# stm233/image-compression-for-machine

Hardware: AMD Instinct MI355X
Metric: images/sec (256x256) cnn-hyperprior (WACNN) training step (higher is better)
Workload: dtype f32; 1 GPU; cnn (WACNN N=192 M=320) train step, lambda=0.0067 MSE, batch 16/GPU synthetic 256x256, Adam lr 1e-4 + aux Adam, clip 1.0; global_batch=16, parallelism=dp1

## Files before the change

### image-compression-for-machine_amd/csrc/conv_wino.hip

```cpp
#include <cmath>
#include <cstdlib>
#include "conv_common.h"

namespace icm {

struct WinoDesc {
  ConvPtrs g[ICM_MAX_GROUPS];
  long long x_bs, y_bs, res_bs, aux_bs, y2_bs;
  int N, Cin, Cout, H, W;
  int lgTX, lgTY, lgTI, tiles_x, tiles_y, tiles_n;
  int ncot, nchunks8, ncb, nsteps;
  int epi, accum, act;
  int seg_len, seg_gap;
  FastDiv dseg;
  int dbg;
  int vpre;
  int px_fast, npx;
};

#define WINO_STEP_FLOATS (2 * 16 * 8 * 32)

template <int EPI>
__device__ __forceinline__ void wino_finish(const WinoDesc& d, const ConvPtrs& P, float v, int co, long long off, bool ok) {
  if (!ok) return;
  if (P.bias) v += P.bias[co];
  float side;
  v = epi_apply<EPI>(v, epi_reads_res(EPI) ? P.res[off] : 0.0f, epi_reads_aux(EPI) ? P.aux[off] : 0.0f, side);
  if constexpr (epi_writes_side(EPI))
    if (P.y2) P.y2[off] = side;
  if (d.accum) v += P.y[off];
  if constexpr (epi_may_gelu(EPI))
    if (P.y2) epi_materialise(v, P.y, P.y2, off, true);
  P.y[off] = v;
}

typedef float f32x2 __attribute__((ext_vector_type(2)));
template <int EPI>
__device__ __forceinline__ void wino_finish2(const WinoDesc& d, const ConvPtrs& P, float v0, float v1, int co, long long off,
                                             bool ok) {
  if (!ok) return;
  if (P.bias) {
    const float b = P.bias[co];
    v0 += b;
    v1 += b;
  }
  f32x2 rv = {0.0f, 0.0f}, av = {0.0f, 0.0f};
  if constexpr (epi_reads_res(EPI)) rv = *reinterpret_cast<const f32x2*>(P.res + off);
  if constexpr (epi_reads_aux(EPI)) av = *reinterpret_cast<const f32x2*>(P.aux + off);
  float s0, s1;
  v0 = epi_apply<EPI>(v0, rv[0], av[0], s0);
  v1 = epi_apply<EPI>(v1, rv[1], av[1], s1);
  if constexpr (epi_writes_side(EPI))
    if (P.y2) *reinterpret_cast<f32x2*>(P.y2 + off) = f32x2{s0, s1};
  if (d.accum) {
    const f32x2 old = *reinterpret_cast<const f32x2*>(P.y + off);
    v0 += old[0];
    v1 += old[1];
  }
  if constexpr (epi_may_gelu(EPI))
    if (P.y2) {
      float g0 = v0, g1 = v1;
      epi_materialise(g0, P.y, P.y, off, false);
      epi_materialise(g1, P.y, P.y, off, false);
      if (P.y2 == P.y) {
        v0 = g0;
        v1 = g1;
      } else {
        *reinterpret_cast<f32x2*>(P.y2 + off) = f32x2{g0, g1};
      }
    }
  *reinterpret_cast<f32x2*>(P.y + off) = f32x2{v0, v1};
}

template <int TCO>
__global__ __launch_bounds__(512, 2) void conv_wino_kernel(const WinoDesc d) {
  extern __shared__ __attribute__((aligned(16))) float smem[];
  const int tid = threadIdx.x, lane = tid & 63;
  const int wave = __builtin_amdgcn_readfirstlane(tid >> 6);
  ConvPtrs P = d.g[blockIdx.y];
  int bid = xcd_block_id();
  const int cb = d.px_fast ? bid / d.npx : bid % d.ncb;
  int pt = d.px_fast ? bid % d.npx : bid / d.ncb;
  const int pblk = pt;
  const int bx = pt % d.tiles_x;
  pt /= d.tiles_x;
  const int by = pt % d.tiles_y;
  const int bn = pt / d.tiles_y;
  const int TXm = (1 << d.lgTX) - 1, TYm = (1 << d.lgTY) - 1;
  const int HW = d.H * d.W;

  if (wave >= 4 && d.vpre) {
    const int lw = wave - 4;
    const float* vsrc = P.x + (long long)pblk * (d.nsteps * 2) * 4096;
    auto dma = [&](int step, int buf) {
#pragma unroll
      for (int k = 0; k < 2; ++k)
#pragma unroll
        for (int rnd = 0; rnd < 4; ++rnd) {
          const int e = (rnd * 256 + lw * 64) * 4;
          __builtin_amdgcn_global_load_lds(vsrc + ((long long)(step * 2 + k) * 4096 + e + lane * 4),
                                           smem + buf * WINO_STEP_FLOATS + k * 4096 + e, 16, 0, 0);
        }
    };
    dma(0, 0);
    asm volatile("s_waitcnt vmcnt(0)" ::: "memory");
    __syncthreads();
    for (int s = 0; s < d.nsteps; ++s) {
      if (s + 1 < d.nsteps) dma(s + 1, (s + 1) & 1);
      asm volatile("s_waitcnt vmcnt(0)" ::: "memory");
      __syncthreads();
    }
  } else if (wave >= 4) {
    const int q = (wave - 4) * 64 + lane;
    const int ci_l = q >> 5, t = q & 31;
    const int tx = t & TXm, ty = (t >> d.lgTX) & TYm, ti = t >> (d.lgTX + d.lgTY);
    const int n = (bn << d.lgTI) + ti;
    const int oy = (((by << d.lgTY) + ty) << 1), ox = (((bx << d.lgTX) + tx) << 1);
    unsigned mask = 0;
#pragma unroll
    for (int dy = 0; dy < 4; ++dy)
#pragma unroll
      for (int dx = 0; dx < 4; ++dx) {
        const int iy = oy - 1 + dy, ix = ox - 1 + dx;
        if (n < d.N && (unsigned)iy < (unsigned)d.H && (unsigned)ix < (unsigned)d.W) mask |= 1u << (dy * 4 + dx);
      }
    const float* xbase = P.x + ((long long)n * d.x_bs + (long long)(oy - 1) * d.W + (ox - 1));
    const int act = d.act;
    auto load = [&](float (&r)[2][16], int step) {
#pragma unroll
      for (int k = 0; k < 2; ++k) {
        const int c = (step * 2 + k) * 8 + ci_l;
        const bool cok = c < d.Cin;
        const int cp = d.seg_len ? c + (int)fdiv((uint32_t)c, d.dseg) * d.seg_gap : c;
        const float* pc = xbase + (long long)cp * HW;
#pragma unroll
        for (int dy = 0; dy < 4; ++dy)
#pragma unroll
          for (int dx = 0; dx < 4; ++dx)
            r[k][dy * 4 + dx] = (cok && ((mask >> (dy * 4 + dx)) & 1u) && !(d.dbg & 1)) ? pc[dy * d.W + dx] : 0.0f;
      }
    };
    auto transform_store = [&](const float (&r)[2][16], int buf) {
      if (d.dbg & 8) return;
#pragma unroll
      for (int k = 0; k < 2; ++k) {
        float dd[16], u[16];
#pragma unroll
        for (int e = 0; e < 16; ++e) dd[e] = act ? apply_act(r[k][e], act) : r[k][e];
#pragma unroll
        for (int j = 0; j < 4; ++j) {
          u[0 * 4 + j] = dd[0 * 4 + j] - dd[2 * 4 + j];
          u[1 * 4 + j] = dd[1 * 4 + j] + dd[2 * 4 + j];
          u[2 * 4 + j] = dd[2 * 4 + j] - dd[1 * 4 + j];
          u[3 * 4 + j] = dd[1 * 4 + j] - dd[3 * 4 + j];
        }
        float* dst = smem + buf * WINO_STEP_FLOATS + k * (16 * 256) + ci_l * 32 + t;
#pragma unroll
        for (int i = 0; i < 4; ++i) {
          dst[(i * 4 + 0) * 256] = u[i * 4 + 0] - u[i * 4 + 2];
          dst[(i * 4 + 1) * 256] = u[i * 4 + 1] + u[i * 4 + 2];
          dst[(i * 4 + 2) * 256] = u[i * 4 + 2] - u[i * 4 + 1];
          dst[(i * 4 + 3) * 256] = u[i * 4 + 1] - u[i * 4 + 3];
        }
      }
    };
    float ra[2][16], rb[2][16], rc[2][16];
    load(ra, 0);
    if (d.nsteps > 1) load(rb, 1);
    if (d.nsteps > 2) load(rc, 2);
    transform_store(ra, 0);
    __syncthreads();
    for (int s = 0; s < d.nsteps; s += 3) {
      if (s + 3 < d.nsteps) load(ra, s + 3);
      if (s + 1 < d.nsteps) transform_store(rb, (s + 1) & 1);
      __syncthreads();
      if (s + 1 >= d.nsteps) break;
      if (s + 4 < d.nsteps) load(rb, s + 4);
      if (s + 2 < d.nsteps) transform_store(rc, (s + 2) & 1);
      __syncthreads();
      if (s + 2 >= d.nsteps) break;
      if (s + 5 < d.nsteps) load(rc, s + 5);
      if (s + 3 < d.nsteps) transform_store(ra, (s + 3) & 1);
      __syncthreads();
    }
  } else {
  const int r = wave;
  f32x16 acc[4][TCO];
  const int cot0 = cb * TCO;
#pragma unroll
  for (int c = 0; c < 4; ++c)
#pragma unroll
    for (int a = 0; a < TCO; ++a)
#pragma unroll
      for (int e = 0; e < 16; ++e) acc[c][a][e] = 0.0f;
  const char* wbase = reinterpret_cast<const char*>(P.wp);
  unsigned wl[TCO];
#pragma unroll
  for (int a = 0; a < TCO; ++a) wl[a] = (unsigned)(min(cot0 + a, d.ncot - 1) * 64 + lane) * 16u;
  const long long qstride = (long long)d.ncot * 64 * 16;
  const int nunits = d.nsteps * 8;
  const int lastq = d.nchunks8 * 16 - 1;
  auto wptr = [&](int g) -> const char* {
    const int qq = min((g >> 2) * 16 + 4 * r + (g & 3), lastq);
    return wbase + qq * qstride;
  };
  f32x4 aq[4][TCO];
#pragma unroll
  for (int u = 0; u < 3; ++u)
#pragma unroll
    for (int a = 0; a < TCO; ++a) aq[u][a] = *reinterpret_cast<const f32x4*>(wptr(u) + wl[a]);
  const int boff = (4 * r) * 256 + lane;
  __syncthreads();
  for (int s = 0; s < d.nsteps; ++s) {
    const float* vb = smem + (s & 1) * WINO_STEP_FLOATS + boff;
    float bv[2][4];
#pragma unroll
    for (int j = 0; j < 4; ++j) bv[0][j] = vb[j * 64];
#pragma unroll
    for (int u = 0; u < 8; ++u) {
      const int g = s * 8 + u;
      if (u + 1 < 8) {
        const float* nb = vb + ((u + 1) >> 2) * (16 * 256) + ((u + 1) & 3) * 256;
#pragma unroll
        for (int j = 0; j < 4; ++j) bv[(u + 1) & 1][j] = (d.dbg & 16) ? 1.0f : nb[j * 64];
      }
      const char* sp = wptr(min(g + 3, nunits - 1));
#pragma unroll
      for (int a = 0; a < TCO; ++a) {
#pragma unroll
        for (int j = 0; j < 4; ++j)
          acc[u & 3][a] = __builtin_amdgcn_mfma_f32_32x32x2f32(aq[u & 3][a][j], bv[u & 1][j], acc[u & 3][a], 0, 0, 0);
        if (!(d.dbg & 2)) aq[(u + 3) & 3][a] = *reinterpret_cast<const f32x4*>(sp + wl[a]);
      }
    }
    __syncthreads();
  }

  float* zb = smem;
#pragma unroll
  for (int a = 0; a < TCO; ++a)
#pragma unroll
    for (int e = 0; e < 16; ++e) {
      const float m0 = acc[0][a][e], m1 = acc[1][a][e], m2 = acc[2][a][e], m3 = acc[3][a][e];
      zb[(((r * 2 + 0) * TCO + a) * 16 + e) * 64 + lane] = (m0 + m1) + m2;
      zb[(((r * 2 + 1) * TCO + a) * 16 + e) * 64 + lane] = (m1 - m2) - m3;
    }
  }
  __syncthreads();
  const float* zb = smem;
  const int cot0 = cb * TCO;
  const int h = lane >> 5, l31 = lane & 31;
  const int tx = l31 & TXm, ty = (l31 >> d.lgTX) & TYm, ti = l31 >> (d.lgTX + d.lgTY);
  const int n = (bn << d.lgTI) + ti;
  const int oy = (((by << d.lgTY) + ty) << 1), ox = (((bx << d.lgTX) + tx) << 1);
  const bool nok = n < d.N;
  P.y += (long long)n * d.y_bs;
  if (P.y2) P.y2 += (long long)n * d.y2_bs;
  if (P.res) P.res += (long long)n * d.res_bs;
  if (P.aux) P.aux += (long long)n * d.aux_bs;
  auto finish_all = [&](auto epi_tag) {
    constexpr int EPI = decltype(epi_tag)::value;
#pragma unroll
    for (int a = 0; a < TCO; ++a) {
      const int cot = cot0 + a;
      if (cot >= d.ncot) continue;
#pragma unroll
      for (int i = 0; i < 2; ++i) {
        const int e = wave + 8 * i;
        const int co = cot * 32 + (e & 3) + 8 * (e >> 2) + 4 * h;
        float z[4][2];
#pragma unroll
        for (int rr = 0; rr < 4; ++rr)
#pragma unroll
          for (int cp = 0; cp < 2; ++cp) z[rr][cp] = zb[(((rr * 2 + cp) * TCO + a) * 16 + e) * 64 + lane];
        const bool cok = nok && co < d.Cout;
        const long long base = (long long)co * HW + (long long)oy * d.W + ox;
#pragma unroll
        for (int cp = 0; cp < 2; ++cp) {
          const float y0 = (z[0][cp] + z[1][cp]) + z[2][cp];
          const float y1 = (z[1][cp] - z[2][cp]) - z[3][cp];
          const bool xok = cok && ox + cp < d.W;
          wino_finish<EPI>(d, P, y0, co, base + cp, xok && oy < d.H);
          wino_finish<EPI>(d, P, y1, co, base + d.W + cp, xok && oy + 1 < d.H);
        }
      }
    }
  };
  if (d.dbg & 4) return;
  EpiWino::dispatch(d.epi, finish_all);
}


template <int TCO>
__global__ __launch_bounds__(512, 2) void conv_wino8_kernel(const WinoDesc d) {
  extern __shared__ __attribute__((aligned(16))) float smem[];
  const int tid = threadIdx.x, lane = tid & 63;
  const int wave = __builtin_amdgcn_readfirstlane(tid >> 6);
  ConvPtrs P = d.g[blockIdx.y];
  int bid = xcd_block_id();
  const int cb = d.px_fast ? bid / d.npx : bid % d.ncb;
  int pt = d.px_fast ? bid % d.npx : bid / d.ncb;
  const int pblk = pt;
  const int bx = pt % d.tiles_x;
  pt /= d.tiles_x;
  const int by = pt % d.tiles_y;
  const int bn = pt / d.tiles_y;
  const int TXm = (1 << d.lgTX) - 1, TYm = (1 << d.lgTY) - 1;
  const int HW = d.H * d.W;
  const int r = wave >> 1, ch = wave & 1;
  const int cot0 = cb * TCO;

  const float* vsrc = P.x + (long long)pblk * (d.nsteps * 2) * 4096;
  auto dma = [&](int step, int buf) {
#pragma unroll
    for (int i = 0; i < 4; ++i) {
      const int piece = wave + 8 * i;
      const int e = (piece >> 4) * 4096 + (piece & 15) * 256;
      __builtin_amdgcn_global_load_lds(vsrc + (long long)step * 8192 + e + lane * 4, smem + buf * WINO_STEP_FLOATS + e, 16, 0, 0);
    }
  };
  f32x16 acc[2][TCO];
#pragma unroll
  for (int c = 0; c < 2; ++c)
#pragma unroll
    for (int a = 0; a < TCO; ++a)
#pragma unroll
      for (int e = 0; e < 16; ++e) acc[c][a][e] = 0.0f;
  const char* wbase = reinterpret_cast<const char*>(P.wp);
  unsigned wl[TCO];
#pragma unroll
  for (int a = 0; a < TCO; ++a) wl[a] = (unsigned)(min(cot0 + a, d.ncot - 1) * 64 + lane) * 16u;
  const long long qstride = (long long)d.ncot * 64 * 16;
  const int nunits = d.nsteps * 4;
  const int lastq = d.nchunks8 * 16 - 1;
  const int xi0 = 4 * r + 2 * ch;
  auto wptr = [&](int g) -> const char* {
    const int qq = min((g >> 1) * 16 + xi0 + (g & 1), lastq);
    return wbase + qq * qstride;
  };
  constexpr int AHEAD = TCO == 3 ? 1 : 2, SLOTM = 2 * AHEAD - 1;
  dma(0, 0);
  if (AHEAD == 2 && d.nsteps > 1) dma(1, 1);
  f32x4 aq[4][TCO];
#pragma unroll
  for (int u = 0; u < 3; ++u)
#pragma unroll
    for (int a = 0; a < TCO; ++a) aq[u][a] = *reinterpret_cast<const f32x4*>(wptr(min(u, nunits - 1)) + wl[a]);
  const int boff = xi0 * 256 + lane;
  asm volatile("s_waitcnt vmcnt(0)" ::: "memory");
  __syncthreads();
  float bv[2][4];
  if constexpr (AHEAD == 2) {
#pragma unroll
    for (int j = 0; j < 4; ++j) bv[0][j] = (smem + boff)[j * 64];
  }
  for (int s = 0; s < d.nsteps; ++s) {
    if (s + AHEAD < d.nsteps) dma(s + AHEAD, (s + AHEAD) & SLOTM);
    const float* vb = smem + (s & SLOTM) * WINO_STEP_FLOATS + boff;
    if constexpr (AHEAD == 1) {
#pragma unroll
      for (int j = 0; j < 4; ++j) bv[0][j] = vb[j * 64];
    }
#pragma unroll
    for (int u = 0; u < 4; ++u) {
      const int g = s * 4 + u;
      if (u + 1 < 4 || AHEAD == 2) {
        const float* nb = u + 1 < 4 ? vb + ((u + 1) >> 1) * (16 * 256) + ((u + 1) & 1) * 256
                                    : smem + ((s + 1) & SLOTM) * WINO_STEP_FLOATS + boff;
#pragma unroll
        for (int j = 0; j < 4; ++j) bv[(u + 1) & 1][j] = nb[j * 64];
      }
      const char* sp = wptr(min(g + 3, nunits - 1));
#pragma unroll
      for (int a = 0; a < TCO; ++a) {
#pragma unroll
        for (int j = 0; j < 4; ++j)
          acc[u & 1][a] = __builtin_amdgcn_mfma_f32_32x32x2f32(aq[u][a][j], bv[u & 1][j], acc[u & 1][a], 0, 0, 0);
        aq[(u + 3) & 3][a] = *reinterpret_cast<const f32x4*>(sp + wl[a]);
      }
    }
    if constexpr (TCO == 4) asm volatile("s_waitcnt vmcnt(12)" ::: "memory");
    else if constexpr (TCO == 3) asm volatile("s_waitcnt vmcnt(9)" ::: "memory");
    else asm volatile("s_waitcnt vmcnt(6)" ::: "memory");
    if constexpr (AHEAD == 1) asm volatile("s_waitcnt lgkmcnt(0)" ::: "memory");
    __builtin_amdgcn_s_barrier();
  }

  float* zb = smem;
  const int h = lane >> 5, l31 = lane & 31;
  const int tx = l31 & TXm, ty = (l31 >> d.lgTX) & TYm, ti = l31 >> (d.lgTX + d.lgTY);
  const int n = (bn << d.lgTI) + ti;
  const int oy = (((by << d.lgTY) + ty) << 1), ox = (((bx << d.lgTX) + tx) << 1);
  const bool nok = n < d.N;
  P.y += (long long)n * d.y_bs;
  if (P.y2) P.y2 += (long long)n * d.y2_bs;
  if (P.res) P.res += (long long)n * d.res_bs;
  if (P.aux) P.aux += (long long)n * d.aux_bs;
  const ConvPtrs& P0 = d.g[blockIdx.y];
  const bool pair = ((d.W | d.y_bs | d.y2_bs | d.res_bs | d.aux_bs) & 1) == 0 &&
                    ((reinterpret_cast<uintptr_t>(P0.y) | reinterpret_cast<uintptr_t>(P0.y2) |
                      reinterpret_cast<uintptr_t>(P0.res) | reinterpret_cast<uintptr_t>(P0.aux)) & 7) == 0;
  auto pass = [&](auto a0_tag) {
    constexpr int a0 = decltype(a0_tag)::value;
    __syncthreads();
#pragma unroll
    for (int al = 0; al < 2; ++al) {
      if (a0 + al >= TCO) break;
#pragma unroll
      for (int e = 0; e < 16; ++e) {
        const float m0 = acc[0][a0 + al][e], m1 = acc[1][a0 + al][e];
        const float p0 = ch == 0 ? m0 + m1 : m0;
        const float p1 = ch == 0 ? m1 : -m0 - m1;
        zb[((((al * 4 + r) * 2 + ch) * 2 + 0) * 16 + e) * 64 + lane] = p0;
        zb[((((al * 4 + r) * 2 + ch) * 2 + 1) * 16 + e) * 64 + lane] = p1;
      }
    }
    __syncthreads();
    auto finish_all = [&](auto epi_tag) {
      constexpr int EPI = decltype(epi_tag)::value;
#pragma unroll
      for (int al = 0; al < 2; ++al) {
        const int cot = cot0 + a0 + al;
        if (a0 + al >= TCO || cot >= d.ncot) continue;
#pragma unroll
        for (int i = 0; i < 2; ++i) {
          const int e = wave + 8 * i;
          const int co = cot * 32 + (e & 3) + 8 * (e >> 2) + 4 * h;
          float z[4][2];
#pragma unroll
          for (int rr = 0; rr < 4; ++rr)
#pragma unroll
            for (int cp = 0; cp < 2; ++cp)
              z[rr][cp] = zb[((((al * 4 + rr) * 2 + 0) * 2 + cp) * 16 + e) * 64 + lane] +
                          zb[((((al * 4 + rr) * 2 + 1) * 2 + cp) * 16 + e) * 64 + lane];
          const bool cok = nok && co < d.Cout;
          const long long base = (long long)co * HW + (long long)oy * d.W + ox;
          float y0[2], y1[2];
#pragma unroll
          for (int cp = 0; cp < 2; ++cp) {
            y0[cp] = (z[0][cp] + z[1][cp]) + z[2][cp];
            y1[cp] = (z[1][cp] - z[2][cp]) - z[3][cp];
          }
          if (pair) {
            const bool xok = cok && ox < d.W;
            wino_finish2<EPI>(d, P, y0[0], y0[1], co, base, xok && oy < d.H);
            wino_finish2<EPI>(d, P, y1[0], y1[1], co, base + d.W, xok && oy + 1 < d.H);
          } else {
#pragma unroll
            for (int cp = 0; cp < 2; ++cp) {
              const bool xok = cok && ox + cp < d.W;
              wino_finish<EPI>(d, P, y0[cp], co, base + cp, xok && oy < d.H);
              wino_finish<EPI>(d, P, y1[cp], co, base + d.W + cp, xok && oy + 1 < d.H);
            }
          }
        }
      }
    };
    EpiWino::dispatch(d.epi, finish_all);
  };
  pass(std::integral_constant<int, 0>{});
  if constexpr (TCO > 2) pass(std::integral_constant<int, 2>{});
}

bool wino_supported(const icm_conv_args& a);

struct WinoXfDesc {
  const float* x[ICM_MAX_GROUPS];
  float* v[ICM_MAX_GROUPS];
  long long x_bs;
  int N, Cin, H, W, lgTX, lgTY, lgTI, tiles_x, tiles_y, nchunks, act, seg_len, seg_gap;
  FastDiv dseg;
};
typedef float f32x4u __attribute__((ext_vector_type(4), aligned(4)));
template <bool VEC>
__global__ __launch_bounds__(256) void wino_input_transform_kernel(const WinoXfDesc d) {
  const float* x = d.x[blockIdx.y];
  float* v = d.v[blockIdx.y];
  const int chunk = blockIdx.x % d.nchunks;
  int pt = blockIdx.x / d.nchunks;
  const int pblk = pt;
  const int bx = pt % d.tiles_x;
  pt /= d.tiles_x;
  const int by = pt % d.tiles_y;
  const int bn = pt / d.tiles_y;
  const int q = threadIdx.x, ci_l = q >> 5, t = q & 31;
  const int TXm = (1 << d.lgTX) - 1, TYm = (1 << d.lgTY) - 1;
  const int tx = t & TXm, ty = (t >> d.lgTX) & TYm, ti = t >> (d.lgTX + d.lgTY);
  const int n = (bn << d.lgTI) + ti;
  const int oy = (((by << d.lgTY) + ty) << 1), ox = (((bx << d.lgTX) + tx) << 1);
  const int c = chunk * 8 + ci_l;
  const bool cok = c < d.Cin && n < d.N;
  const int cp = d.seg_len ? c + (int)fdiv((uint32_t)c, d.dseg) * d.seg_gap : c;
  const long long pbase = (long long)n * d.x_bs + (long long)cp * d.H * d.W + (long long)(oy - 1) * d.W + (ox - 1);
  float dd[16], u[16];
  if constexpr (VEC) {
    const bool tvalid = cok && ox < d.W;
    const bool left = ox == 0, right = ox == d.W - 2;
    f32x4u rv[4];
    bool rok[4];
#pragma unroll
    for (int dy = 0; dy < 4; ++dy) {
      rok[dy] = tvalid && (unsigned)(oy - 1 + dy) < (unsigned)d.H;
      const long long off = rok[dy] ? pbase + dy * d.W + (left ? 1 : (right ? -1 : 0)) : 0;
      rv[dy] = *reinterpret_cast<const f32x4u*>(x + off);
    }
#pragma unroll
    for (int dy = 0; dy < 4; ++dy) {
      const f32x4u w4 = rv[dy];
      float e[4];
      e[0] = left ? 0.0f : (right ? w4[1] : w4[0]);
      e[1] = left ? w4[0] : (right ? w4[2] : w4[1]);
      e[2] = left ? w4[1] : (right ? w4[3] : w4[2]);
      e[3] = left ? w4[2] : (right ? 0.0f : w4[3]);
#pragma unroll
      for (int dx = 0; dx < 4; ++dx) {
        const float val = rok[dy] ? e[dx] : 0.0f;
        dd[dy * 4 + dx] = d.act ? apply_act(val, d.act) : val;
      }
    }
  } else {
    const float* pc = x + pbase;
#pragma unroll
    for (int dy = 0; dy < 4; ++dy)
#pragma unroll
      for (int dx = 0; dx < 4; ++dx) {
        const int iy = oy - 1 + dy, ix = ox - 1 + dx;
        const float val = (cok && (unsigned)iy < (unsigned)d.H && (unsigned)ix < (unsigned)d.W) ? pc[dy * d.W + dx] : 0.0f;
        dd[dy * 4 + dx] = d.act ? apply_act(val, d.act) : val;
      }
  }
#pragma unroll
  for (int j = 0; j < 4; ++j) {
    u[0 * 4 + j] = dd[0 * 4 + j] - dd[2 * 4 + j];
    u[1 * 4 + j] = dd[1 * 4 + j] + dd[2 * 4 + j];
    u[2 * 4 + j] = dd[2 * 4 + j] - dd[1 * 4 + j];
    u[3 * 4 + j] = dd[1 * 4 + j] - dd[3 * 4 + j];
  }
  float* dst = v + ((long long)pblk * d.nchunks + chunk) * 4096 + ci_l * 32 + t;
#pragma unroll
  for (int i = 0; i < 4; ++i) {
    dst[(i * 4 + 0) * 256] = u[i * 4 + 0] - u[i * 4 + 2];
    dst[(i * 4 + 1) * 256] = u[i * 4 + 1] + u[i * 4 + 2];
    dst[(i * 4 + 2) * 256] = u[i * 4 + 2] - u[i * 4 + 1];
    dst[(i * 4 + 3) * 256] = u[i * 4 + 1] - u[i * 4 + 3];
  }
}

static WinoGeom wino_geometry(const icm_conv_args& a) {
  WinoGeom g;
  const int tw = cdiv(a.W, 2), th = cdiv(a.H, 2);
  g.lgTX = std::min(3, ceil_log2(tw));
  g.lgTY = std::min(5 - g.lgTX, ceil_log2(th));
  g.lgTI = 5 - g.lgTX - g.lgTY;
  g.tiles_x = cdiv(tw, 1 << g.lgTX); g.tiles_y = cdiv(th, 1 << g.lgTY); g.tiles_n = cdiv(a.N, 1 << g.lgTI);
  g.nchunks8 = cdiv(a.Cin, 8); g.nsteps = cdiv(g.nchunks8, 2);
  return g;
}

long long wino_transform_floats(const icm_conv_args& a) {
  const WinoGeom g = wino_geometry(a);
  return (long long)g.tiles_x * g.tiles_y * g.tiles_n * (g.nsteps * 2) * 4096;
}

int run_wino_transform(const icm_conv_args* arr, int ngroups, hipStream_t stream) {
  const icm_conv_args& a = arr[0];
  if (!wino_supported(a)) return ICM_ERR_UNSUPPORTED;
  const WinoGeom g = wino_geometry(a);
  WinoXfDesc d{};
  for (int gi = 0; gi < ICM_MAX_GROUPS; ++gi) {
    const icm_conv_args& s = arr[gi < ngroups ? gi : 0];
    if (!s.x || !s.xv) return ICM_ERR_ARG;
    d.x[gi] = s.x; d.v[gi] = s.xv;
  }
  d.x_bs = a.x_bs; d.N = a.N; d.Cin = a.Cin; d.H = a.H; d.W = a.W;
  d.lgTX = g.lgTX; d.lgTY = g.lgTY; d.lgTI = g.lgTI; d.tiles_x = g.tiles_x; d.tiles_y = g.tiles_y;
  d.nchunks = g.nsteps * 2; d.act = a.pro_act;
  d.seg_len = a.x_seg_len; d.seg_gap = a.x_seg_len ? a.x_seg_gap : 0;
  d.dseg = make_fastdiv((uint32_t)std::max(1, a.x_seg_len));
  const long long nblk = (long long)g.tiles_x * g.tiles_y * g.tiles_n * d.nchunks;
  if (nblk <= 0 || nblk > 0x7fffffffLL) return ICM_ERR_ARG;
  static const bool novec = env_int("ICM_WINO_XF_NOVEC", 0) != 0;
  if (!novec && a.W % 2 == 0 && a.W >= 4)
    hipLaunchKernelGGL(wino_input_transform_kernel<true>, dim3((unsigned)nblk, ngroups), dim3(256), 0, stream, d);
  else
    hipLaunchKernelGGL(wino_input_transform_kernel<false>, dim3((unsigned)nblk, ngroups), dim3(256), 0, stream, d);
  ICM_CHECK_LAUNCH();
  return ICM_OK;
}

bool wino_supported(const icm_conv_args& a) {
  if (a.KH != 3 || a.KW != 3 || a.stride != 1 || a.pad != 1 || a.pixel_shuffle) return false;
  if (a.OH != a.H || a.OW != a.W) return false;
  if (!EpiWino::has(a.epi)) return false;
  if (a.pro_act != ICM_ACT_NONE && a.pro_act != ICM_ACT_GELU && a.pro_act != ICM_ACT_SQUARE) return false;
  return true;
}

int plan_conv_wino(const icm_conv_args& a, int ngroups, WinoPlan& p) {
  if (!wino_supported(a)) return ICM_ERR_UNSUPPORTED;
  p.g = wino_geometry(a);
  const int ncot = cdiv(a.Cout, 32);
  const long long pblocks = (long long)p.g.tiles_x * p.g.tiles_y * p.g.tiles_n;
  static const int force_tco = env_int("ICM_WINO_TCO", 0);
  int tco = 2;
  {
    const long long b2 = pblocks * cdiv(ncot, 2) * ngroups, b1 = pblocks * ncot * ngroups;
    const double t2 = std::ceil(b2 / 256.0) * 2.0, t1 = std::ceil(b1 / 256.0) * 1.0 * 1.08;
    if (ncot == 1 || t1 < t2) tco = 1;
    if (force_tco == 1 || force_tco == 2) tco = force_tco;
  }
  static const int w8_on = env_int("ICM_WINO8", 1);
  bool w8 = a.xv != nullptr && w8_on;
  if (w8) {
    int t8 = 2;
    double bestc = 1e300;
    for (int t = 4; t >= 2; --t) {
      const long long b = pblocks * cdiv(ncot, t) * ngroups;
      const double c = std::ceil(b / 256.0) * (t + 0.6);
      if (c < bestc - 1e-9) { bestc = c; t8 = t; }
    }
    if (force_tco >= 2 && force_tco <= 4) t8 = force_tco;
    static const long long w8_min = env_ll("ICM_WINO8_MINWG", 150);
    if (pblocks * cdiv(ncot, t8) * ngroups >= w8_min || force_tco >= 2) tco = t8;
    else w8 = false;
  }
  p.tco = tco; p.w8 = w8; p.ncb = cdiv(ncot, tco);
  const double wbytes = 64.0 * a.Cin * a.Cout, abytes = 4.0 * a.Cin * a.N * a.H * a.W;
  static const int force_order = env_int("ICM_WINO_PXFAST", -1);
  p.px_fast = (force_order == 0 || force_order == 1) ? force_order : ((wbytes > 3.0e6 && wbytes > abytes) ? 1 : 0);
  p.nblk = pblocks * p.ncb;
  if (p.nblk <= 0 || p.nblk > 0x7fffffffLL) return ICM_ERR_ARG;
  p.lds_bytes = w8 ? (size_t)2 * 4 * 2 * 2 * 16 * 64 * sizeof(float) : (size_t)2 * WINO_STEP_FLOATS * sizeof(float);
  return ICM_OK;
}

int run_conv_wino(const icm_conv_args* arr, int ngroups, hipStream_t stream) {
  const icm_conv_args& a = arr[0];
  WinoPlan p;
  if (int rc = plan_conv_wino(a, ngroups, p)) return rc;
  WinoDesc d{};
  fill_conv_ptrs(d.g, arr, ngroups, 0);
  d.x_bs = a.x_bs; d.y_bs = a.y_bs; d.res_bs = a.res_bs; d.aux_bs = a.aux_bs; d.y2_bs = a.y2_bs;
  d.N = a.N; d.Cin = a.Cin; d.Cout = a.Cout; d.H = a.H; d.W = a.W;
  d.lgTX = p.g.lgTX; d.lgTY = p.g.lgTY; d.lgTI = p.g.lgTI; d.tiles_x = p.g.tiles_x; d.tiles_y = p.g.tiles_y; d.tiles_n = p.g.tiles_n;
  d.nchunks8 = p.g.nchunks8; d.nsteps = p.g.nsteps;
  d.ncot = cdiv(a.Cout, 32);
  d.vpre = a.xv != nullptr ? 1 : 0;
  if (d.vpre)
    for (int gi = 0; gi < ICM_MAX_GROUPS; ++gi) {
      const icm_conv_args& s = arr[gi < ngroups ? gi : 0];
      if (!s.xv) return ICM_ERR_ARG;
      d.g[gi].x = s.xv;
    }
  d.epi = a.epi; d.accum = a.accum; d.act = a.pro_act;
  d.seg_len = a.x_seg_len; d.seg_gap = a.x_seg_len ? a.x_seg_gap : 0;
  d.dseg = make_fastdiv((uint32_t)std::max(1, a.x_seg_len));
  d.ncb = p.ncb; d.npx = (int)(p.nblk / p.ncb); d.px_fast = p.px_fast;
  static const int dbg = env_int("ICM_WINO_DEBUG", 0);
  d.dbg = dbg;
  void (*fn)(const WinoDesc) = p.tco == 2 ? conv_wino_kernel<2> : conv_wino_kernel<1>;
  if (p.w8) {
    fn = p.tco == 4 ? conv_wino8_kernel<4> : (p.tco == 3 ? conv_wino8_kernel<3> : conv_wino8_kernel<2>);
    if (!ensure_max_lds(reinterpret_cast<const void*>(fn))) return ICM_ERR_LAUNCH;
  }
  hipLaunchKernelGGL(fn, dim3((unsigned)p.nblk, ngroups, 1), dim3(512), p.lds_bytes, stream, d);
  ICM_CHECK_LAUNCH();
  return ICM_OK;
}

}
```

Before: 396.4 images/s.

## Hand-schedule Winograd weight loads with inline asm and explicit vmcnt waits

Replaces compiler-generated weight prefetch loads in the Winograd MFMA main loop with inline-asm global_load_dwordx4 and precise s_waitcnt vmcnt counts per sub-step. The prologue no longer drains every outstanding load before the first barrier. The TCO=3 variant now also uses a two-step-ahead LDS DMA pipeline instead of one. The aim is to stop the compiler inserting conservative full waits, so weight and activation loads overlap better with MFMA work. The cost is fragile hand-counted vmcnt values that can cause races if the counts are wrong.

```diff
diff --git a/image-compression-for-machine_amd/csrc/conv_wino.hip b/image-compression-for-machine_amd/csrc/conv_wino.hip
--- a/image-compression-for-machine_amd/csrc/conv_wino.hip
+++ b/image-compression-for-machine_amd/csrc/conv_wino.hip
@@ -292,6 +292,44 @@
 
 
 template <int TCO>
+struct Wino8Pipe {
+  static constexpr int AHEAD = 2;
+  static constexpr int SLOTM = 2 * AHEAD - 1;
+  static constexpr int W_PROLOGUE = 3 * TCO;
+  static constexpr int W_EDGE = 2 * TCO;
+  static constexpr int W_MID = 2 * TCO + 4;
+  static constexpr int W_BARRIER = 4 * TCO;
+};
+
+template <int TCO>
+__device__ __forceinline__ void wino8_wload(f32x4 (&q)[TCO], const char* base, const unsigned (&wl)[TCO]) {
+  if constexpr (TCO == 2)
+    asm volatile("s_nop 4\n\tglobal_load_dwordx4 %0, %2, %4\n\tglobal_load_dwordx4 %1, %3, %4"
+                 : "=&v"(q[0]), "=&v"(q[1]) : "v"(wl[0]), "v"(wl[1]), "s"(base) : "memory");
+  else if constexpr (TCO == 3)
+    asm volatile("s_nop 4\n\tglobal_load_dwordx4 %0, %3, %6\n\tglobal_load_dwordx4 %1, %4, %6\n\tglobal_load_dwordx4 %2, %5, %6"
+                 : "=&v"(q[0]), "=&v"(q[1]), "=&v"(q[2]) : "v"(wl[0]), "v"(wl[1]), "v"(wl[2]), "s"(base) : "memory");
+  else
+    asm volatile("s_nop 4\n\tglobal_load_dwordx4 %0, %4, %8\n\tglobal_load_dwordx4 %1, %5, %8\n\t"
+                 "global_load_dwordx4 %2, %6, %8\n\tglobal_load_dwordx4 %3, %7, %8"
+                 : "=&v"(q[0]), "=&v"(q[1]), "=&v"(q[2]), "=&v"(q[3])
+                 : "v"(wl[0]), "v"(wl[1]), "v"(wl[2]), "v"(wl[3]), "s"(base) : "memory");
+}
+template <int N, int TCO>
+__device__ __forceinline__ void wino8_wwait(f32x4 (&q)[TCO]) {
+  if constexpr (TCO == 2)
+    asm volatile("s_waitcnt vmcnt(%2)\n\ts_nop 1" : "+v"(q[0]), "+v"(q[1]) : "n"(N) : "memory");
+  else if constexpr (TCO == 3)
+    asm volatile("s_waitcnt vmcnt(%3)\n\ts_nop 1" : "+v"(q[0]), "+v"(q[1]), "+v"(q[2]) : "n"(N) : "memory");
+  else
+    asm volatile("s_waitcnt vmcnt(%4)\n\ts_nop 1" : "+v"(q[0]), "+v"(q[1]), "+v"(q[2]), "+v"(q[3]) : "n"(N) : "memory");
+}
+template <int N>
+__device__ __forceinline__ void wino8_vmwait() {
+  asm volatile("s_waitcnt vmcnt(%0)" ::"n"(N) : "memory");
+}
+
+template <int TCO>
 __global__ __launch_bounds__(512, 2) void conv_wino8_kernel(const WinoDesc d) {
   extern __shared__ __attribute__((aligned(16))) float smem[];
   const int tid = threadIdx.x, lane = tid & 63;
@@ -309,6 +347,8 @@
   const int HW = d.H * d.W;
   const int r = wave >> 1, ch = wave & 1;
   const int cot0 = cb * TCO;
+  using PL = Wino8Pipe<TCO>;
+  constexpr int AHEAD = PL::AHEAD, SLOTM = PL::SLOTM;
 
   const float* vsrc = P.x + (long long)pblk * (d.nsteps * 2) * 4096;
   auto dma = [&](int step, int buf) {
@@ -338,53 +378,53 @@
     const int qq = min((g >> 1) * 16 + xi0 + (g & 1), lastq);
     return wbase + qq * qstride;
   };
-  constexpr int AHEAD = TCO == 3 ? 1 : 2, SLOTM = 2 * AHEAD - 1;
   dma(0, 0);
-  if (AHEAD == 2 && d.nsteps > 1) dma(1, 1);
+  if (d.nsteps > 1) dma(1, 1);
   f32x4 aq[4][TCO];
 #pragma unroll
-  for (int u = 0; u < 3; ++u)
-#pragma unroll
-    for (int a = 0; a < TCO; ++a) aq[u][a] = *reinterpret_cast<const f32x4*>(wptr(min(u, nunits - 1)) + wl[a]);
+  for (int u = 0; u < 3; ++u) wino8_wload<TCO>(aq[u], wptr(min(u, nunits - 1)), wl);
   const int boff = xi0 * 256 + lane;
-  asm volatile("s_waitcnt vmcnt(0)" ::: "memory");
-  __syncthreads();
+  wino8_vmwait<PL::W_PROLOGUE>();
+  __builtin_amdgcn_s_barrier();
   float bv[2][4];
-  if constexpr (AHEAD == 2) {
-#pragma unroll
-    for (int j = 0; j < 4; ++j) bv[0][j] = (smem + boff)[j * 64];
-  }
+#pragma unroll
+  for (int j = 0; j < 4; ++j) bv[0][j] = (smem + boff)[j * 64];
   for (int s = 0; s < d.nsteps; ++s) {
-    if (s + AHEAD < d.nsteps) dma(s + AHEAD, (s + AHEAD) & SLOTM);
+    const bool more = s + AHEAD < d.nsteps;
     const float* vb = smem + (s & SLOTM) * WINO_STEP_FLOATS + boff;
-    if constexpr (AHEAD == 1) {
-#pragma unroll
-      for (int j = 0; j < 4; ++j) bv[0][j] = vb[j * 64];
-    }
 #pragma unroll
     for (int u = 0; u < 4; ++u) {
       const int g = s * 4 + u;
-      if (u + 1 < 4 || AHEAD == 2) {
-        const float* nb = u + 1 < 4 ? vb + ((u + 1) >> 1) * (16 * 256) + ((u + 1) & 1) * 256
-                                    : smem + ((s + 1) & SLOTM) * WINO_STEP_FLOATS + boff;
-#pragma unroll
-        for (int j = 0; j < 4; ++j) bv[(u + 1) & 1][j] = nb[j * 64];
-      }
-      const char* sp = wptr(min(g + 3, nunits - 1));
-#pragma unroll
-      for (int a = 0; a < TCO; ++a) {
+      if (u == 0 || u == 3) {
+        wino8_wwait<PL::W_EDGE>(aq[u]);
+      } else {
+        if (!more) wino8_vmwait<PL::W_EDGE>();
+        wino8_wwait<PL::W_MID>(aq[u]);
+      }
+      if (u == 0 && more) dma(s + AHEAD, (s + AHEAD) & SLOTM);
+      wino8_wload<TCO>(aq[(u + 3) & 3], wptr(min(g + 3, nunits - 1)), wl);
+      const float* nb = u + 1 < 4 ? vb + ((u + 1) >> 1) * (16 * 256) + ((u + 1) & 1) * 256
+                                  : smem + ((s + 1) & SLOTM) * WINO_STEP_FLOATS + boff;
+#pragma unroll
+      for (int j = 0; j < 4; ++j) bv[(u + 1) & 1][j] = nb[j * 64];
+#pragma unroll
+      for (int a = 0; a < TCO; ++a)
 #pragma unroll
         for (int j = 0; j < 4; ++j)
           acc[u & 1][a] = __builtin_amdgcn_mfma_f32_32x32x2f32(aq[u][a][j], bv[u & 1][j], acc[u & 1][a], 0, 0, 0);
-        aq[(u + 3) & 3][a] = *reinterpret_cast<const f32x4*>(sp + wl[a]);
-      }
-    }
-    if constexpr (TCO == 4) asm volatile("s_waitcnt vmcnt(12)" ::: "memory");
-    else if constexpr (TCO == 3) asm volatile("s_waitcnt vmcnt(9)" ::: "memory");
-    else asm volatile("s_waitcnt vmcnt(6)" ::: "memory");
-    if constexpr (AHEAD == 1) asm volatile("s_waitcnt lgkmcnt(0)" ::: "memory");
+    }
+    wino8_vmwait<PL::W_BARRIER>();
     __builtin_amdgcn_s_barrier();
   }
+  if constexpr (TCO == 2)
+    asm volatile("s_waitcnt vmcnt(0)" : "+v"(aq[0][0]), "+v"(aq[0][1]), "+v"(aq[1][0]), "+v"(aq[1][1]), "+v"(aq[2][0]), "+v"(aq[2][1])
+                 :: "memory");
+  else if constexpr (TCO == 3)
+    asm volatile("s_waitcnt vmcnt(0)" : "+v"(aq[0][0]), "+v"(aq[0][1]), "+v"(aq[0][2]), "+v"(aq[1][0]), "+v"(aq[1][1]), "+v"(aq[1][2]),
+                   "+v"(aq[2][0]), "+v"(aq[2][1]), "+v"(aq[2][2]) :: "memory");
+  else
+    asm volatile("s_waitcnt vmcnt(0)" : "+v"(aq[0][0]), "+v"(aq[0][1]), "+v"(aq[0][2]), "+v"(aq[0][3]), "+v"(aq[1][0]), "+v"(aq[1][1]),
+                   "+v"(aq[1][2]), "+v"(aq[1][3]), "+v"(aq[2][0]), "+v"(aq[2][1]), "+v"(aq[2][2]), "+v"(aq[2][3]) :: "memory");
 
   float* zb = smem;
   const int h = lane >> 5, l31 = lane & 31;
```

Result: faster. 405.3 images/s, median of 6 (+2.2%).
